# atenpas/gpd

Hardware: AMD Instinct MI355X
Metric: 15-ch grasp candidates scored/sec (imagegen+LeNet) at 1/2/4/8 MI355X (higher is better)
Workload: dtype f64 geometry / u8 images / LeNet f32-equivalent by exact operand splitting: conv1 int8 digit planes of 32-bit fixed-point weights (i32 accumulate, exact), conv2 + ip1 three bf16 pieces per operand (six exact products per term, f32 accumulate), ip2 f32

## Files before the change

gpd_amd/csrc/lenet_fast.hip:

```cpp
#include "gpd_internal.h"
#include "buffers.h"

#include <cstring>

namespace gpd {

typedef int i32x4 __attribute__((ext_vector_type(4)));
typedef float f32x4 __attribute__((ext_vector_type(4)));
typedef __bf16 bf16x8 __attribute__((ext_vector_type(8)));
typedef unsigned int u32x4 __attribute__((ext_vector_type(4)));

constexpr int F1_THREADS = 512, F1_WAVES = 8;
constexpr int F1_PITCH = 72;
constexpr int F1_ROWB = F1_PITCH * 16;
constexpr int F1_HWC = kImg * F1_ROWB;
constexpr int F1_TILES = 28 * 7;
constexpr int F1_KS = 7, F1_MT = 5;

__host__ __device__ constexpr int f1_tap(int ks, int g) {
  return ks < 5 ? ((g == 0 ? 0 : g == 1 ? 2 : g == 2 ? 1 : 3) * 5 + ks) : ks == 5 ? 20 + g : (g == 0 ? 24 : -1);
}
constexpr int F1P_KS = 5;
constexpr int F1P_ROWB = 736;
constexpr int F1P_COPY = kImg * F1P_ROWB;
constexpr int F1N_KS = 3;
constexpr int F1N_PITCH = 68;
constexpr int F1N_COPY = kImg * F1N_PITCH * 4;
__host__ __device__ constexpr int f1n_slot(int ks, int g) {
  const int sl = 4 * ks + g;
  return sl < 5 ? 2 * sl : sl < 10 ? 2 * (sl - 5) + 1 : -1;
}

__device__ inline double max_f64(double a, double b) {
  double r;
  asm("v_max_f64 %0, %1, %2" : "=v"(r) : "v"(a), "v"(b));
  return r;
}
__device__ inline double dpp_quad_max(double v) {
  int lo = __double2loint(v), hi = __double2hiint(v);
  double o = __hiloint2double(__builtin_amdgcn_mov_dpp(hi, 0xB1, 0xf, 0xf, true), __builtin_amdgcn_mov_dpp(lo, 0xB1, 0xf, 0xf, true));
  v = max_f64(v, o);
  lo = __double2loint(v);
  hi = __double2hiint(v);
  o = __hiloint2double(__builtin_amdgcn_mov_dpp(hi, 0x4E, 0xf, 0xf, true), __builtin_amdgcn_mov_dpp(lo, 0x4E, 0xf, 0xf, true));
  return max_f64(v, o);
}

template <int C, bool RELU>
__device__ __forceinline__ void conv1_i8_body(const uint8_t *__restrict__ images, const uint4 *__restrict__ atab,
                                              const double *__restrict__ corr, const int *__restrict__ shift,
                                              const float *__restrict__ bias, float *__restrict__ pool1, int n,
                                              int *__restrict__ queue) {
  constexpr int RAW = C * kPix, NV = RAW / 16;
  static_assert(RAW % 16 == 0 && C <= 16, "image bytes");
  constexpr bool NARROW = C <= 4;
  constexpr bool PACK12 = C == 12;
  constexpr int KS = NARROW ? F1N_KS : PACK12 ? F1P_KS : F1_KS;
  __shared__ __attribute__((aligned(16))) uint8_t s_hwc[NARROW ? 4 * F1N_COPY : PACK12 ? 2 * F1P_COPY : F1_HWC];
  __shared__ __attribute__((aligned(16))) uint8_t s_raw[RAW];
  __shared__ int s_nxt;
  const int tid = threadIdx.x, lane = tid & 63;
  const int wave = __builtin_amdgcn_readfirstlane(tid >> 6);
  const int j = lane & 15, q = lane >> 4;
  int img = blockIdx.x;
  if (img >= n) return;
  if (wave < F1_WAVES / 2) __builtin_amdgcn_s_setprio(2);
  i32x4 A[KS][F1_MT];
#pragma unroll
  for (int ks = 0; ks < KS; ks++)
#pragma unroll
    for (int mt = 0; mt < F1_MT; mt++) {
      const uint4 v = atab[(ks * F1_MT + mt) * 64 + lane];
      A[ks][mt] = i32x4{(int)v.x, (int)v.y, (int)v.z, (int)v.w};
    }
  {
    const uint4 *src = reinterpret_cast<const uint4 *>(images + (size_t)img * RAW);
    uint4 *dst = reinterpret_cast<uint4 *>(s_raw);
    for (int i = tid; i < NV; i += F1_THREADS) dst[i] = src[i];
  }
  __syncthreads();
  auto transpose = [&]() {
    if constexpr (NARROW) {
      for (int task = tid; task < kImg * (kImg / 4); task += F1_THREADS) {
        const int y = task / (kImg / 4), x0 = 4 * (task - y * (kImg / 4));
        uint32_t r[4];
#pragma unroll
        for (int c = 0; c < 4; c++) r[c] = c < C ? *reinterpret_cast<const uint32_t *>(s_raw + c * kPix + y * kImg + x0) : 0x80808080u;
        const uint32_t t0 = __builtin_amdgcn_perm(r[1], r[0], 0x05010400u), t1 = __builtin_amdgcn_perm(r[1], r[0], 0x07030602u);
        const uint32_t t2 = __builtin_amdgcn_perm(r[3], r[2], 0x05010400u), t3 = __builtin_amdgcn_perm(r[3], r[2], 0x07030602u);
        const uint32_t o0 = __builtin_amdgcn_perm(t2, t0, 0x05040100u) ^ 0x80808080u, o1 = __builtin_amdgcn_perm(t2, t0, 0x07060302u) ^ 0x80808080u;
        const uint32_t o2 = __builtin_amdgcn_perm(t3, t1, 0x05040100u) ^ 0x80808080u, o3 = __builtin_amdgcn_perm(t3, t1, 0x07060302u) ^ 0x80808080u;
        uint8_t *d = s_hwc + (y * F1N_PITCH + x0) * 4;
        *reinterpret_cast<uint4 *>(d) = make_uint4(o0, o1, o2, o3);
#pragma unroll
        for (int sh = 1; sh < 4; sh++) {
          uint32_t *e = reinterpret_cast<uint32_t *>(d + sh * F1N_COPY + sh * 4);
          e[0] = o0;
          e[1] = o1;
          e[2] = o2;
          e[3] = o3;
        }
      }
      return;
    }
    if constexpr (PACK12) {
      for (int task = tid; task < kImg * (kImg / 4); task += F1_THREADS) {
        const int y = task / (kImg / 4), x0 = 4 * (task - y * (kImg / 4));
        uint32_t o[4][3];
#pragma unroll
        for (int cg = 0; cg < 3; cg++) {
          uint32_t r[4];
#pragma unroll
          for (int c = 0; c < 4; c++) r[c] = *reinterpret_cast<const uint32_t *>(s_raw + (4 * cg + c) * kPix + y * kImg + x0);
          const uint32_t t0 = __builtin_amdgcn_perm(r[1], r[0], 0x05010400u), t1 = __builtin_amdgcn_perm(r[1], r[0], 0x07030602u);
          const uint32_t t2 = __builtin_amdgcn_perm(r[3], r[2], 0x05010400u), t3 = __builtin_amdgcn_perm(r[3], r[2], 0x07030602u);
          o[0][cg] = __builtin_amdgcn_perm(t2, t0, 0x05040100u) ^ 0x80808080u;
          o[1][cg] = __builtin_amdgcn_perm(t2, t0, 0x07060302u) ^ 0x80808080u;
          o[2][cg] = __builtin_amdgcn_perm(t3, t1, 0x05040100u) ^ 0x80808080u;
          o[3][cg] = __builtin_amdgcn_perm(t3, t1, 0x07060302u) ^ 0x80808080u;
        }
        uint8_t *d = s_hwc + y * F1P_ROWB + 12 * x0;
        uint4 *d4 = reinterpret_cast<uint4 *>(d);
        d4[0] = make_uint4(o[0][0], o[0][1], o[0][2], o[1][0]);
        d4[1] = make_uint4(o[1][1], o[1][2], o[2][0], o[2][1]);
        d4[2] = make_uint4(o[2][2], o[3][0], o[3][1], o[3][2]);
        uint32_t *e = reinterpret_cast<uint32_t *>(d + F1P_COPY + 4);
#pragma unroll
        for (int px = 0; px < 4; px++)
#pragma unroll
          for (int cg = 0; cg < 3; cg++) e[3 * px + cg] = o[px][cg];
      }
      return;
    }
    for (int task = tid; task < kImg * (kImg / 4); task += F1_THREADS) {
      const int y = task / (kImg / 4), x0 = 4 * (task - y * (kImg / 4));
      uint32_t r[16];
#pragma unroll
      for (int c = 0; c < 16; c++) r[c] = c < C ? *reinterpret_cast<const uint32_t *>(s_raw + c * kPix + y * kImg + x0) : 0u;
      uint32_t o[4][4];
#pragma unroll
      for (int cg = 0; cg < 4; cg++) {
        const uint32_t t0 = __builtin_amdgcn_perm(r[4 * cg + 1], r[4 * cg], 0x05010400u);
        const uint32_t t1 = __builtin_amdgcn_perm(r[4 * cg + 1], r[4 * cg], 0x07030602u);
        const uint32_t t2 = __builtin_amdgcn_perm(r[4 * cg + 3], r[4 * cg + 2], 0x05010400u);
        const uint32_t t3 = __builtin_amdgcn_perm(r[4 * cg + 3], r[4 * cg + 2], 0x07030602u);
        o[0][cg] = __builtin_amdgcn_perm(t2, t0, 0x05040100u) ^ 0x80808080u;
        o[1][cg] = __builtin_amdgcn_perm(t2, t0, 0x07060302u) ^ 0x80808080u;
        o[2][cg] = __builtin_amdgcn_perm(t3, t1, 0x05040100u) ^ 0x80808080u;
        o[3][cg] = __builtin_amdgcn_perm(t3, t1, 0x07060302u) ^ 0x80808080u;
      }
#pragma unroll
      for (int e = 0; e < 4; e++)
        *reinterpret_cast<uint4 *>(s_hwc + (y * F1_PITCH + x0 + e) * 16) = make_uint4(o[e][0], o[e][1], o[e][2], o[e][3]);
    }
  };
  transpose();
  const int m_row = (j >> 1) & 1, m_x = 2 * (j >> 2) + (j & 1);
  const int kyg = q == 0 ? 0 : q == 1 ? 2 : q == 2 ? 1 : 3;
  const int n_shift = (4 - (m_x & 3)) & 3;
  const int lane_off = NARROW   ? n_shift * F1N_COPY + (m_row * F1N_PITCH + m_x + n_shift) * 4
                       : PACK12 ? (m_x & 1) * (F1P_COPY + 4) + m_row * F1P_ROWB + 12 * m_x + 16 * q
                                : (m_row * F1_PITCH + m_x) * 16;
  int n_slot[F1N_KS];
#pragma unroll
  for (int ks = 0; ks < F1N_KS; ks++) {
    const int sl = q == 0 ? f1n_slot(ks, 0) : q == 1 ? f1n_slot(ks, 1) : q == 2 ? f1n_slot(ks, 2) : f1n_slot(ks, 3);
    n_slot[ks] = sl < 0 ? 0 : ((sl >> 1) * F1N_PITCH + 4 * (sl & 1)) * 4;
  }
  const int p = j & 3, w = j >> 2;
  const double k_corr_own = corr[4 * p + q], k_corr_4 = corr[16 + q];
  const int k_shift_own = shift[4 * p + q], k_shift_4 = shift[16 + q];
  const float k_bias_own = bias[4 * p + q], k_bias_4 = bias[16 + q];
  for (;;) {
    if (tid == 0) s_nxt = (int)gridDim.x + atomicAdd(queue, 1);
    __syncthreads();
    const int nxt = s_nxt;
    const uint4 *nsrc = reinterpret_cast<const uint4 *>(images + (size_t)(nxt < n ? nxt : img) * RAW);
    auto tile_addr = [&](int t, const uint8_t *&pa, const uint8_t *&pb, const uint8_t *&pc) {
      const int tc = t < F1_TILES ? t : F1_TILES - 1;
      const int trow = tc / 7, tcol = tc - 7 * trow;
      if constexpr (NARROW) {
        pa = pb = pc = s_hwc + ((2 * trow) * F1N_PITCH + 8 * tcol) * 4 + lane_off;
      } else if constexpr (PACK12) {
        pa = pb = pc = s_hwc + (2 * trow) * F1P_ROWB + 12 * (8 * tcol) + lane_off;
      } else {
        const uint8_t *base = s_hwc + ((2 * trow) * F1_PITCH + 8 * tcol) * 16 + lane_off;
        pa = base + kyg * F1_ROWB;
        pb = base + 4 * F1_ROWB + q * 16;
        pc = base + 4 * F1_ROWB + 4 * 16;
      }
    };
    auto frag_b = [&](int ks, const uint8_t *pa, const uint8_t *pb, const uint8_t *pc) {
      if constexpr (NARROW) return *reinterpret_cast<const i32x4 *>(pa + n_slot[ks < F1N_KS ? ks : 0]);
      else if constexpr (PACK12) {
        typedef const volatile __attribute__((address_space(3))) unsigned long long *lds_u64;
        const unsigned long long lo = *(lds_u64)(pa + ks * F1P_ROWB), hi = *(lds_u64)(pa + ks * F1P_ROWB + 8);
        return i32x4{(int)(uint32_t)lo, (int)(uint32_t)(lo >> 32), (int)(uint32_t)hi, (int)(uint32_t)(hi >> 32)};
      }
      else return *reinterpret_cast<const i32x4 *>(ks < 5 ? pa + ks * 16 : ks == 5 ? pb : pc);
    };
    i32x4 B[KS];
    {
      const uint8_t *pa, *pb, *pc;
      tile_addr(wave, pa, pb, pc);
#pragma unroll
      for (int ks = 0; ks < KS; ks++) B[ks] = frag_b(ks, pa, pb, pc);
    }
    int it = 0;
    for (int t = wave; t < F1_TILES; t += F1_WAVES, it++) {
      const int piece = it * F1_THREADS + tid;
      const bool has_piece = nxt < n && piece < NV;
      uint4 stage = make_uint4(0, 0, 0, 0);
      if (has_piece) stage = nsrc[piece];
      i32x4 acc[F1_MT];
#pragma unroll
      for (int mt = 0; mt < F1_MT; mt++) acc[mt] = i32x4{0, 0, 0, 0};
      __builtin_amdgcn_sched_barrier(0);
#pragma unroll
      for (int ks = 0; ks < KS; ks++)
#pragma unroll
        for (int mt = 0; mt < F1_MT; mt++) acc[mt] = __builtin_amdgcn_mfma_i32_16x16x64_i8(A[ks][mt], B[ks], acc[mt], 0, 0, 0);
      __builtin_amdgcn_sched_barrier(0);
      {
        const uint8_t *pa, *pb, *pc;
        tile_addr(t + F1_WAVES, pa, pb, pc);
#pragma unroll
        for (int ks = 0; ks < KS; ks++) B[ks] = frag_b(ks, pa, pb, pc);
      }
      __builtin_amdgcn_sched_barrier(0);
      double sm[F1_MT];
#pragma unroll
      for (int mt = 0; mt < F1_MT; mt++) {
        const int hi = (int)((unsigned)acc[mt][3] << 8) + acc[mt][2];
        const int lo = (int)((unsigned)acc[mt][1] << 8) + acc[mt][0];
        sm[mt] = dpp_quad_max(__builtin_fma((double)hi, 65536.0, (double)lo));
      }
      const double s_own = p == 0 ? sm[0] : p == 1 ? sm[1] : p == 2 ? sm[2] : sm[3];
      float v_own = ldexpf((float)(s_own + k_corr_own), -k_shift_own) + k_bias_own;
      float v_4 = ldexpf((float)(sm[4] + k_corr_4), -k_shift_4) + k_bias_4;
      if constexpr (RELU) {
        v_own = fmaxf(v_own, 0.f);
        v_4 = fmaxf(v_4, 0.f);
      }
      const int trow = t / 7, tcol = t - 7 * trow;
      float *dst = pool1 + ((size_t)img * 784 + trow * 28 + 4 * tcol + w) * 20;
      dst[4 * p + q] = v_own;
      if (p == 0) dst[16 + q] = v_4;
      if (has_piece) reinterpret_cast<uint4 *>(s_raw)[piece] = stage;
    }
    __syncthreads();
    if (nxt >= n) break;
    transpose();
    img = nxt;
  }
}

template <int C>
__global__ __launch_bounds__(F1_THREADS) void conv1_i8_kernel(const uint8_t *__restrict__ images,
                                                              const uint4 *__restrict__ atab, const double *__restrict__ corr,
                                                              const int *__restrict__ shift, const float *__restrict__ bias,
                                                              float *__restrict__ pool1, int n, int *__restrict__ queue) {
  conv1_i8_body<C, false>(images, atab, corr, shift, bias, pool1, n, queue);
}
template <int C>
__global__ __launch_bounds__(F1_THREADS) void conv1_i8_relu_kernel(const uint8_t *__restrict__ images,
                                                                   const uint4 *__restrict__ atab,
                                                                   const double *__restrict__ corr,
                                                                   const int *__restrict__ shift,
                                                                   const float *__restrict__ bias, float *__restrict__ pool1,
                                                                   int n, int *__restrict__ queue) {
  conv1_i8_body<C, true>(images, atab, corr, shift, bias, pool1, n, queue);
}

__device__ inline bf16x8 as_bf16x8(const uint4 &v) {
  bf16x8 r;
  __builtin_memcpy(&r, &v, 16);
  return r;
}

struct Bf3 {
  unsigned short h, m, l;
};
__host__ __device__ inline unsigned short bf16_bits(float x) {
#if defined(__HIP_DEVICE_COMPILE__)
  const __bf16 b = (__bf16)x;
  unsigned short u;
  __builtin_memcpy(&u, &b, 2);
  return u;
#else
  uint32_t u;
  memcpy(&u, &x, 4);
  if ((u & 0x7f800000u) == 0x7f800000u) return (unsigned short)((u >> 16) | ((u & 0xffffu) ? 0x40u : 0u));
  u += 0x7fffu + ((u >> 16) & 1u);
  return (unsigned short)(u >> 16);
#endif
}
__host__ __device__ inline float bf16_value(unsigned short b) {
  const uint32_t u = (uint32_t)b << 16;
  float f;
#if defined(__HIP_DEVICE_COMPILE__)
  __builtin_memcpy(&f, &u, 4);
#else
  memcpy(&f, &u, 4);
#endif
  return f;
}
__host__ __device__ inline Bf3 bf16_split3(float a) {
  Bf3 r;
  r.h = bf16_bits(a);
  const float r1 = a - bf16_value(r.h);
  r.m = bf16_bits(r1);
  const float r2 = r1 - bf16_value(r.m);
  r.l = bf16_bits(r2);
  return r;
}

constexpr int F2_THREADS = 512;
constexpr int F2_PP = 28 * 40;
constexpr int F2_RS = 3 * F2_PP;
constexpr int F2_IMG = 28 * F2_RS;
constexpr int F2_RAW = 784 * 20 * 4;
constexpr int F2_LUNITS = 24;
constexpr int F2_XLD = kLenetXld;

constexpr int F3_KSTEPS = F2_XLD / 32;
__host__ __device__ inline size_t f3_blocked(int r, int k, int pc) {
  const int rr = r & 15;
  return ((((size_t)(r >> 4) * F3_KSTEPS + (k >> 5)) * 3 + pc) << 10) + rr * 64 + ((((k >> 3) & 3) ^ ((4 - (rr >> 2)) & 3)) << 4) + (k & 7) * 2;
}

__host__ __device__ constexpr int f2_slot_tap(int e, int g) {
  return e < 25 ? (e / 5) * 5 + g : e < 30 ? g * 5 + 4 : e == 30 ? 24 : (g == 0 ? 24 : -1);
}
__host__ __device__ constexpr int f2_slot_cg(int e, int g) { return e < 25 ? e % 5 : e < 30 ? e - 25 : e == 30 ? g : 4; }

template <bool RELU>
__device__ __forceinline__ void conv2_bf16_body(const float *__restrict__ pool1, const uint4 *__restrict__ btab,
                                                const float *__restrict__ bias, unsigned short *__restrict__ xs, int n,
                                                int *__restrict__ queue) {
  __shared__ __attribute__((aligned(16))) uint8_t s_img[F2_IMG];
  __shared__ __attribute__((aligned(16))) uint8_t s_raw[F2_RAW];
  __shared__ int s_nxt;
  const int tid = threadIdx.x, lane = tid & 63;
  const int wave = __builtin_amdgcn_readfirstlane(tid >> 6);
  const int j = lane & 15, q = lane >> 4;
  const int img0 = blockIdx.x;
  if (img0 >= n) return;
  {
    const uint4 *src = reinterpret_cast<const uint4 *>(pool1 + (size_t)img0 * (784 * 20));
    uint4 *dst = reinterpret_cast<uint4 *>(s_raw);
    for (int i = tid; i < F2_RAW / 16; i += F2_THREADS) dst[i] = src[i];
  }
  __syncthreads();
  auto split = [&]() {
    for (int task = tid; task < 784 * 5; task += F2_THREADS) {
      const int px = task / 5, cg = task - 5 * px;
      const int row = px / 28, col = px - 28 * row;
      const float4 a = *reinterpret_cast<const float4 *>(s_raw + px * 80 + cg * 16);
      const Bf3 s0 = bf16_split3(a.x), s1 = bf16_split3(a.y), s2 = bf16_split3(a.z), s3 = bf16_split3(a.w);
      uint8_t *d = s_img + row * F2_RS + col * 40 + cg * 8;
      *reinterpret_cast<uint2 *>(d) = make_uint2(s0.h | ((uint32_t)s1.h << 16), s2.h | ((uint32_t)s3.h << 16));
      *reinterpret_cast<uint2 *>(d + F2_PP) = make_uint2(s0.m | ((uint32_t)s1.m << 16), s2.m | ((uint32_t)s3.m << 16));
      *reinterpret_cast<uint2 *>(d + 2 * F2_PP) = make_uint2(s0.l | ((uint32_t)s1.l << 16), s2.l | ((uint32_t)s3.l << 16));
    }
  };
  split();
  auto store_x = [&](int img, int pixel, int f, float v) {
    const Bf3 sp = bf16_split3(v);
    uint8_t *o = reinterpret_cast<uint8_t *>(xs) + f3_blocked(img, pixel * 50 + f, 0);
    *reinterpret_cast<unsigned short *>(o) = sp.h;
    *reinterpret_cast<unsigned short *>(o + 1024) = sp.m;
    *reinterpret_cast<unsigned short *>(o + 2048) = sp.l;
  };
  auto image_loop = [&](int passes, auto carries, auto &&work) {
    int img = img0;
    for (;;) {
      if (tid == 0) s_nxt = (int)gridDim.x + atomicAdd(queue, 1);
      __syncthreads();
      const int nxt = s_nxt;
      const uint4 *nsrc = reinterpret_cast<const uint4 *>(pool1 + (size_t)(nxt < n ? nxt : img) * (784 * 20));
#pragma unroll 1
      for (int tt = 0; tt < passes; tt++) {
        const int piece = tt * (7 * 64) + tid;
        const bool has_piece = decltype(carries)::value && nxt < n && piece < F2_RAW / 16;
        uint4 stage = make_uint4(0, 0, 0, 0);
        if (has_piece) stage = nsrc[piece];
        work(img, tt);
        if (has_piece) reinterpret_cast<uint4 *>(s_raw)[piece] = stage;
      }
      __syncthreads();
      if (nxt >= n) break;
      split();
      img = nxt;
    }
  };
  if (wave == 7) {
    __builtin_amdgcn_s_setprio(3);
    bf16x8 LW[3][4];
#pragma unroll
    for (int pc = 0; pc < 3; pc++)
#pragma unroll
      for (int ks = 0; ks < 4; ks++) LW[pc][ks] = as_bf16x8(btab[((3 * 3 + pc) * 16 + ks) * 64 + lane]);
    int l_lo[4], l_hi[4];
#pragma unroll
    for (int ks = 0; ks < 4; ks++) {
      const int idx = min(4 * ks + q, 14), ky = idx / 3, c8 = idx - 3 * ky;
      l_lo[ks] = ky * F2_RS + j * 40 + c8 * 16;
      l_hi[ks] = c8 == 2 ? l_lo[ks] : l_lo[ks] + 8;
    }
    const int f_own = 48 + (q & 1);
    const float k_bias = bias[f_own];
    auto unit_base = [&](int u) { return s_img + (2 * (u >> 1)) * F2_RS + (12 * (u & 1)) * 40; };
    auto lfrag = [&](const uint8_t *ubase, int step, int pc) -> bf16x8 {
      typedef const volatile __attribute__((address_space(3))) unsigned long long *lds_u64;
      const uint8_t *a = ubase + (step >> 2) * F2_RS + pc * F2_PP;
      const unsigned long long lo = *(lds_u64)(a + l_lo[step & 3]), hi = *(lds_u64)(a + l_hi[step & 3]);
      return as_bf16x8(make_uint4((uint32_t)lo, (uint32_t)(lo >> 32), (uint32_t)hi, (uint32_t)(hi >> 32)));
    };
    bf16x8 b_buf[4][3];
    auto shl = [](float v, auto n) {
      return __builtin_bit_cast(float, __builtin_amdgcn_update_dpp(0, __builtin_bit_cast(int, v), 0x100 + decltype(n)::value, 0xf, 0xf, true));
    };
    asm volatile("" ::"v"(k_bias));
    image_loop(F2_LUNITS, std::false_type(), [&](int img, int tt) {
      const uint8_t *ubase = unit_base(tt), *unext = unit_base(tt < F2_LUNITS - 1 ? tt + 1 : tt);
      if (tt == 0) {
#pragma unroll
        for (int st = 0; st < 3; st++)
#pragma unroll
          for (int pc = 0; pc < 3; pc++) b_buf[st][pc] = lfrag(ubase, st, pc);
      }
      f32x4 lacc[2][2] = {{f32x4{0.f, 0.f, 0.f, 0.f}, f32x4{0.f, 0.f, 0.f, 0.f}}, {f32x4{0.f, 0.f, 0.f, 0.f}, f32x4{0.f, 0.f, 0.f, 0.f}}};
#pragma unroll
      for (int step = 0; step < 8; step++) {
#pragma unroll
        for (int pc = 0; pc < 3; pc++) b_buf[(step + 3) & 3][pc] = step + 3 < 8 ? lfrag(ubase, step + 3, pc) : lfrag(unext, step + 3 - 8, pc);
#pragma unroll
        for (int term = 0; term < 6; term++) {
          const int pa = term == 0 ? 2 : (term == 2 || term == 3) ? 1 : 0;
          const int pw = term == 1 ? 2 : (term == 2 || term == 4) ? 1 : 0;
          lacc[step >> 2][term & 1] = __builtin_amdgcn_mfma_f32_16x16x32_bf16(LW[pw][step & 3], b_buf[step & 3][pa], lacc[step >> 2][term & 1], 0, 0, 0);
        }
      }
      float conv_row[2];
#pragma unroll
      for (int rr = 0; rr < 2; rr++) {
        const f32x4 t = lacc[rr][0] + lacc[rr][1];
        const float v = ((t[0] + shl(t[1], std::integral_constant<int, 1>())) + shl(t[2], std::integral_constant<int, 2>())) + shl(t[3], std::integral_constant<int, 3>());
        conv_row[rr] = v + __shfl(shl(t[0], std::integral_constant<int, 4>()), (lane + 32) & 63);
      }
      float pv = fmaxf(conv_row[0], conv_row[1]);
      pv = fmaxf(pv, shl(pv, std::integral_constant<int, 1>())) + k_bias;
      if constexpr (RELU) pv = fmaxf(pv, 0.f);
      if (q < 2 && (j & 1) == 0 && j < 12) store_x(img, (tt >> 1) * 12 + 6 * (tt & 1) + (j >> 1), f_own, pv);
    });
    return;
  }
  const int grp = wave < 4 ? 1 + (wave >> 1) : 0;
  const int t0 = wave == 3 ? 20 : wave < 4 ? 18 * (wave & 1) : 12 * (wave - 4), tcnt = wave == 2 ? 20 : wave == 3 ? 16 : wave < 4 ? 18 : 12;
  bf16x8 W[3][16];
#pragma unroll
  for (int pc = 0; pc < 3; pc++)
#pragma unroll
    for (int ks = 0; ks < 16; ks++) W[pc][ks] = as_bf16x8(btab[((grp * 3 + pc) * 16 + ks) * 64 + lane]);
  const int m_row = (j >> 1) & 1, m_x = 2 * (j >> 2) + (j & 1);
  const int lane_off = m_row * F2_RS + m_x * 40;
  const int off_x = lane_off + 40 * q, off_y = lane_off + q * F2_RS + 4 * 40, off_z = lane_off + 4 * F2_RS + 4 * 40 + 8 * q,
            off_w = lane_off + 4 * F2_RS + 4 * 40 + 32;
  const int f_own = 16 * grp + j;
  const float k_bias = bias[f_own];
  auto tile_base = [&](int tt) {
    const int T = t0 + tt, rp = T / 3, xt = T - 3 * rp;
    return s_img + (2 * rp) * F2_RS + (8 * xt) * 40;
  };
  auto frag = [&](const uint8_t *base, int ks, int pc) -> bf16x8 {
    uint2 v[2];
#pragma unroll
    for (int h = 0; h < 2; h++) {
      const int e = ks + 16 * h;
      const uint8_t *a = e < 25 ? base + off_x + (e / 5) * F2_RS + (e % 5) * 8
                         : e < 30 ? base + off_y + (e - 25) * 8
                         : e == 30 ? base + off_z
                                   : base + off_w;
      typedef const volatile __attribute__((address_space(3))) unsigned long long *lds_u64;
      const unsigned long long t = *(lds_u64)(a + pc * F2_PP);
      v[h] = make_uint2((uint32_t)t, (uint32_t)(t >> 32));
    }
    return as_bf16x8(make_uint4(v[0].x, v[0].y, v[1].x, v[1].y));
  };
  bf16x8 a_buf[2][3];
  image_loop(tcnt, std::true_type(), [&](int img, int tt) {
    if (tt == 0) {
#pragma unroll
      for (int pc = 0; pc < 3; pc++) a_buf[0][pc] = frag(tile_base(0), 0, pc);
    }
    const int T = t0 + tt, rp = T / 3, xt = T - 3 * rp;
    const uint8_t *base = tile_base(tt), *base_next = tile_base(tt < tcnt - 1 ? tt + 1 : tt);
    f32x4 acc[2] = {f32x4{0.f, 0.f, 0.f, 0.f}, f32x4{0.f, 0.f, 0.f, 0.f}};
#pragma unroll
    for (int ks = 0; ks < 16; ks++) {
#pragma unroll
      for (int pc = 0; pc < 3; pc++) a_buf[(ks + 1) & 1][pc] = ks + 1 < 16 ? frag(base, ks + 1, pc) : frag(base_next, 0, pc);
#pragma unroll
      for (int term = 0; term < 6; term++) {
        const int pa = term == 0 ? 2 : (term == 2 || term == 3) ? 1 : 0;
        const int pw = term == 1 ? 2 : (term == 2 || term == 4) ? 1 : 0;
        acc[term & 1] = __builtin_amdgcn_mfma_f32_16x16x32_bf16(a_buf[ks & 1][pa], W[pw][ks], acc[term & 1], 0, 0, 0);
      }
    }
    const f32x4 t = acc[0] + acc[1];
    float pv = fmaxf(fmaxf(t[0], t[1]), fmaxf(t[2], t[3])) + k_bias;
    if constexpr (RELU) pv = fmaxf(pv, 0.f);
    store_x(img, rp * 12 + 4 * xt + q, f_own, pv);
  });
}

__global__ __launch_bounds__(F2_THREADS) void conv2_bf16_kernel(const float *__restrict__ pool1,
                                                                const uint4 *__restrict__ btab, const float *__restrict__ bias,
                                                                unsigned short *__restrict__ xs, int n,
                                                                int *__restrict__ queue) {
  conv2_bf16_body<false>(pool1, btab, bias, xs, n, queue);
}
__global__ __launch_bounds__(F2_THREADS) void conv2_bf16_relu_kernel(const float *__restrict__ pool1,
                                                                     const uint4 *__restrict__ btab,
                                                                     const float *__restrict__ bias,
                                                                     unsigned short *__restrict__ xs, int n,
                                                                     int *__restrict__ queue) {
  conv2_bf16_body<true>(pool1, btab, bias, xs, n, queue);
}

constexpr int F3_THREADS = 512, F3_BN = 256, F3_BK = 32, F3_KQ = 4;
constexpr int F3_KLEN = F2_XLD / F3_KQ, F3_STEPS = F3_KLEN / F3_BK;
static_assert(F2_XLD % (F3_KQ * F3_BK) == 0 && F2_XLD >= kFc1In, "K quarters");
static_assert(F3_STEPS % 2 == 1, "the step loop below runs in pairs + one");

typedef const __attribute__((address_space(1))) void *glds_src_t;
typedef __attribute__((address_space(3))) void *glds_dst_t;

template <int NT>
__global__ __launch_bounds__(F3_THREADS) void fc1_bf16_kernel(const unsigned short *__restrict__ xs, const unsigned short *__restrict__ wt,
                                                             float *__restrict__ out_p, int n) {
  constexpr int BM = 32 * NT;
  constexpr int XB = BM * 64, WB = F3_BN * 64;
  constexpr int STAGE = 3 * (XB + WB);
  __shared__ __attribute__((aligned(16))) uint8_t smem_a[STAGE];
  __shared__ __attribute__((aligned(16))) uint8_t smem_b[STAGE];
  static_assert(2 * STAGE <= 160 * 1024, "LDS");
  const int tid = threadIdx.x;
  const int L = blockIdx.x;
  const int xcd = L & 7;
  const int ut = xcd & 1, kq = xcd >> 1;
  const int m0 = (L >> 3) * BM;
  if (m0 >= n) return;
  const int u0 = ut * F3_BN, k_base = kq * F3_KLEN;
  const int wave = __builtin_amdgcn_readfirstlane(tid >> 6), lane = tid & 63;
  const int wm = wave >> 2, wu = wave & 3;
  const int g = lane >> 4, j = lane & 15;
  constexpr int XBLK = 6 * NT, X_PW = (XBLK + 7) / 8;
  constexpr size_t ROWBLK = (size_t)F3_KSTEPS * 3 * 1024;
  const uint8_t *wsrc[2];
#pragma unroll
  for (int i = 0; i < 2; i++)
    wsrc[i] = reinterpret_cast<const uint8_t *>(wt) + (size_t)(u0 / 16 + wave + 8 * i) * ROWBLK + (size_t)(k_base / 32) * 3072 + lane * 16;
  const uint8_t *xsrc[X_PW];
  int xdst[X_PW];
#pragma unroll
  for (int i = 0; i < X_PW; i++) {
    const int e = min(wave + 8 * i, XBLK - 1), rb = e / 3, pc = e - 3 * rb;
    xsrc[i] = reinterpret_cast<const uint8_t *>(xs) + (size_t)min(m0 / 16 + rb, (n - 1) / 16) * ROWBLK + (size_t)(k_base / 32) * 3072 + pc * 1024 + lane * 16;
    xdst[i] = pc * XB + rb * 1024;
  }
  auto fetch = [&](int step, uint8_t *b) {
    const int so = step * 3072;
#pragma unroll
    for (int pc = 0; pc < 3; pc++)
#pragma unroll
      for (int i = 0; i < 2; i++)
        __builtin_amdgcn_global_load_lds((glds_src_t)(wsrc[i] + so + pc * 1024), (glds_dst_t)(b + 3 * XB + pc * WB + (wave + 8 * i) * 1024), 16, 0, 0);
#pragma unroll
    for (int i = 0; i < X_PW; i++)
      if (wave + 8 * i < XBLK) __builtin_amdgcn_global_load_lds((glds_src_t)(xsrc[i] + so), (glds_dst_t)(b + xdst[i]), 16, 0, 0);
  };
  f32x4 acc[NT][4];
#pragma unroll
  for (int t = 0; t < NT; t++)
#pragma unroll
    for (int c = 0; c < 4; c++) acc[t][c] = f32x4{0.f, 0.f, 0.f, 0.f};
  const int foff = j * 64 + ((g ^ ((4 - (j >> 2)) & 3)) << 4);
  const int xoff = (wm * 16 * NT) * 64 + foff, woff = (wu * 64) * 64 + foff;
  auto compute = [&](const uint8_t *b) {
    bf16x8 wb[3][4], xa[2][NT];
    auto ldw = [&](int pc) {
#pragma unroll
      for (int c = 0; c < 4; c++) wb[pc][c] = as_bf16x8(*reinterpret_cast<const uint4 *>(b + 3 * XB + pc * WB + woff + c * 16 * 64));
    };
    auto ldx = [&](int s, int pa) {
#pragma unroll
      for (int t = 0; t < NT; t++) xa[s][t] = as_bf16x8(*reinterpret_cast<const uint4 *>(b + pa * XB + xoff + t * 16 * 64));
    };
    auto mul = [&](int s, int pw) {
#pragma unroll
      for (int t = 0; t < NT; t++)
#pragma unroll
        for (int c = 0; c < 4; c++) acc[t][c] = __builtin_amdgcn_mfma_f32_16x16x32_bf16(xa[s][t], wb[pw][c], acc[t][c], 0, 0, 0);
    };
    ldw(0);
    ldx(0, 2);
    ldw(1);
    ldx(1, 1);
    __builtin_amdgcn_sched_barrier(0);
    mul(0, 0);
    __builtin_amdgcn_sched_barrier(0);
    ldw(2);
    ldx(0, 0);
    __builtin_amdgcn_sched_barrier(0);
    mul(1, 1);
    mul(1, 0);
    __builtin_amdgcn_sched_barrier(0);
    mul(0, 2);
    mul(0, 1);
    mul(0, 0);
  };
  fetch(0, smem_a);
  __syncthreads();
  for (int t = 0; t < F3_STEPS - 1; t += 2) {
    fetch(t + 1, smem_b);
    __builtin_amdgcn_sched_barrier(0);
    compute(smem_a);
    __syncthreads();
    fetch(t + 2, smem_a);
    __builtin_amdgcn_sched_barrier(0);
    compute(smem_b);
    __syncthreads();
  }
  compute(smem_a);
#pragma unroll
  for (int c = 0; c < 4; c++) {
    const int u = u0 + 64 * wu + 16 * c + j;
    if (u >= kFc1Out) continue;
#pragma unroll
    for (int t = 0; t < NT; t++) {
      const int m = m0 + 16 * NT * wm + 16 * t + 4 * g;
      if (m < n) *reinterpret_cast<f32x4 *>(out_p + fc1p_index(m, kq, u)) = acc[t][c];
    }
  }
}

void lenet_fast_free(LeNetFast &f) {
  device_release(f.c1a, f.c1corr, f.c1shift, f.c2b, f.f1wt);
  f = LeNetFast();
}

void lenet_fast_conv1_tables(int channels, const float *w, std::vector<uint8_t> &atab, std::vector<double> &corr, std::vector<int> &shift) {
  const int K = channels * 25;
  std::vector<long long> W((size_t)20 * K);
  corr.assign(20, 0.0);
  shift.assign(20, 0);
  for (int f = 0; f < 20; f++) {
    float mx = 0.f;
    for (int k = 0; k < K; k++) mx = std::fmax(mx, std::fabs(w[(size_t)f * K + k]));
    int s = 0;
    if (mx > 0.f) {
      int e;
      (void)std::frexp(mx, &e);
      s = 30 - e;
    }
    shift[f] = s;
    long long sum = 0;
    for (int k = 0; k < K; k++) {
      const long long v = std::llrint(std::ldexp((double)w[(size_t)f * K + k], s));
      W[(size_t)f * K + k] = v;
      sum += v;
    }
    corr[f] = 128.0 * (double)sum;
  }
  atab.assign((size_t)F1_KS * F1_MT * 64 * 16, 0);
  auto digit_of = [](long long v, int digit) {
    int d = 0;
    for (int q = 0; q <= digit; q++) {
      d = (int)(((v + 128) & 255) - 128);
      v = (v - d) >> 8;
    }
    return d;
  };
  const bool narrow = channels <= 4;
  const bool pack12 = channels == 12;
  for (int ks = 0; ks < (narrow ? F1N_KS : pack12 ? F1P_KS : F1_KS); ks++)
    for (int mt = 0; mt < F1_MT; mt++)
      for (int lane = 0; lane < 64; lane++) {
        const int i = lane & 15, g = lane >> 4;
        const int f = 4 * mt + (i >> 2), digit = i & 3;
        uint8_t *row = &atab[((size_t)(ks * F1_MT + mt) * 64 + lane) * 16];
        if (narrow) {
          const int sl = f1n_slot(ks, g);
          if (sl < 0) continue;
          const int ky = sl >> 1, half = sl & 1;
          for (int px = 0; px < 4; px++) {
            const int kx = 4 * half + px;
            if (kx > 4) continue;
            for (int c = 0; c < channels; c++) row[4 * px + c] = (uint8_t)(int8_t)digit_of(W[(size_t)f * K + c * 25 + ky * 5 + kx], digit);
          }
          continue;
        }
        if (pack12) {
          for (int b = 0; b < 16; b++) {
            const int kb = 16 * g + b;
            if (kb >= 60) continue;
            row[b] = (uint8_t)(int8_t)digit_of(W[(size_t)f * K + (kb % 12) * 25 + ks * 5 + kb / 12], digit);
          }
          continue;
        }
        const int tap = f1_tap(ks, g);
        if (tap < 0) continue;
        for (int c = 0; c < channels; c++) row[c] = (uint8_t)(int8_t)digit_of(W[(size_t)f * K + c * 25 + tap], digit);
      }
}

void lenet_fast_conv2_tables(const float *w, std::vector<unsigned short> &btab) {
  btab.assign((size_t)4 * 3 * 16 * 64 * 8, 0);
  auto put = [&](int slot, int ks, int lane, int e, float v) {
    const Bf3 sp = bf16_split3(v);
    const unsigned short pcs[3] = {sp.h, sp.m, sp.l};
    for (int pc = 0; pc < 3; pc++) btab[((((size_t)slot * 3 + pc) * 16 + ks) * 64 + lane) * 8 + e] = pcs[pc];
  };
  for (int slot = 0; slot < 3; slot++)
    for (int ks = 0; ks < 16; ks++)
      for (int lane = 0; lane < 64; lane++) {
        const int f = 16 * slot + (lane & 15), g = lane >> 4;
        for (int h = 0; h < 2; h++) {
          const int e = ks + 16 * h, tap = f2_slot_tap(e, g), cg = f2_slot_cg(e, g);
          if (tap < 0) continue;
          for (int c = 0; c < 4; c++) put(slot, ks, lane, 4 * h + c, w[(size_t)f * 500 + (4 * cg + c) * 25 + tap]);
        }
      }
  for (int ks = 0; ks < 4; ks++)
    for (int lane = 0; lane < 64; lane++) {
      const int row = lane & 15, chunk = 4 * ks + (lane >> 4);
      if ((row > 8 && row != 12) || chunk > 14) continue;
      const int f = row < 8 ? 48 + (row >> 2) : 48 + ((row - 8) >> 2), kx = row < 8 ? (row & 3) : 4;
      const int ky = chunk / 3, c0 = 8 * (chunk % 3);
      for (int e = 0; e < 8 && c0 + e < 20; e++) put(3, ks, lane, e, w[(size_t)f * 500 + (c0 + e) * 25 + ky * 5 + kx]);
    }
}

void lenet_fast_ip1_tables(const float *w, std::vector<unsigned short> &wt) {
  wt.assign((size_t)3 * 512 * F2_XLD, 0);
  uint8_t *base = reinterpret_cast<uint8_t *>(wt.data());
  for (int k = 0; k < kFc1In; k++)
    for (int u = 0; u < kFc1Out; u++) {
      const Bf3 sp = bf16_split3(w[(size_t)k * kFc1Out + u]);
      const unsigned short pcs[3] = {sp.h, sp.m, sp.l};
      for (int pc = 0; pc < 3; pc++) memcpy(base + f3_blocked(u, k, pc), &pcs[pc], 2);
    }
}

void lenet_fast_unblock_x(const unsigned short *blocked, int n, unsigned short *planes) {
  const uint8_t *base = reinterpret_cast<const uint8_t *>(blocked);
  for (int pc = 0; pc < 3; pc++)
    for (int m = 0; m < n; m++)
      for (int k = 0; k < kFc1In; k++) memcpy(planes + ((size_t)pc * n + m) * kFc1In + k, base + f3_blocked(m, k, pc), 2);
}

}

extern "C" int gpd_hip_lenet_fast_tables(int channels, const float *c1w, const float *c2w, uint8_t *atab, double *corr, int *shift,
                                         unsigned short *btab) {
  if (!c1w || !c2w || !atab || !corr || !shift || !btab || channels < 1 || channels > 16) return GPD_ERR_INVALID;
  std::vector<uint8_t> a;
  std::vector<double> c;
  std::vector<int> sh;
  std::vector<unsigned short> b;
  gpd::lenet_fast_conv1_tables(channels, c1w, a, c, sh);
  gpd::lenet_fast_conv2_tables(c2w, b);
  memcpy(atab, a.data(), a.size());
  memcpy(corr, c.data(), c.size() * sizeof(double));
  memcpy(shift, sh.data(), sh.size() * sizeof(int));
  memcpy(btab, b.data(), b.size() * sizeof(unsigned short));
  return GPD_OK;
}

namespace gpd {

hipError_t lenet_fast_prepare(LeNetFast &f, int channels, const float *c1w, const float *c2w, const float *f1w) {
  lenet_fast_free(f);
  std::vector<uint8_t> atab;
  std::vector<double> corr;
  std::vector<int> shift;
  std::vector<unsigned short> btab, wt;
  lenet_fast_conv1_tables(channels, c1w, atab, corr, shift);
  lenet_fast_conv2_tables(c2w, btab);
  lenet_fast_ip1_tables(f1w, wt);
  hipError_t e;
  auto up = [&](auto *&dst, const void *src, size_t bytes) -> hipError_t {
    if ((e = device_alloc(dst, (bytes + sizeof(*dst) - 1) / sizeof(*dst))) != hipSuccess) return e;
    return hipMemcpy(dst, src, bytes, hipMemcpyHostToDevice);
  };
  if ((e = up(f.c1a, atab.data(), atab.size())) != hipSuccess) return e;
  if ((e = up(f.c1corr, corr.data(), corr.size() * sizeof(double))) != hipSuccess) return e;
  if ((e = up(f.c1shift, shift.data(), shift.size() * sizeof(int))) != hipSuccess) return e;
  if ((e = up(f.c2b, btab.data(), btab.size() * sizeof(unsigned short))) != hipSuccess) return e;
  if ((e = up(f.f1wt, wt.data(), wt.size() * sizeof(unsigned short))) != hipSuccess) return e;
  return hipSuccess;
}

template <int NT>
static void fc1f_launch(const LeNetWeights &w, LeNetScratch &s, int n, hipStream_t stream) {
  const int m_tiles = (n + 32 * NT - 1) / (32 * NT);
  fc1_bf16_kernel<NT><<<m_tiles * 8, F3_THREADS, 0, stream>>>(s.xs, w.fast.f1wt, s.fc1p, n);
}
static int fc1f_pick_nt(int n) {
  for (int r = 1;; r++) {
    const int nt = (n + 32 * r * 32 - 1) / (32 * r * 32);
    if (nt <= 5) return nt < 1 ? 1 : nt;
  }
}

hipError_t lenet_forward_fast(const LeNetWeights &w, LeNetScratch &s, const uint8_t *img, int m, float *d_scores, hipStream_t stream,
                              hipEvent_t *kernel_events, int *queue) {
  const int num_cus = s.num_cus;
  const int grid = m < num_cus ? m : num_cus;
#define F1_LAUNCH(KERNEL, CH) KERNEL<CH><<<grid, F1_THREADS, 0, stream>>>(img, w.fast.c1a, w.fast.c1corr, w.fast.c1shift, w.c1b, s.pool1, m, queue)
  if (w.conv_relu) {
    switch (w.channels) {
      case 15: F1_LAUNCH(conv1_i8_relu_kernel, 15); break;
      case 12: F1_LAUNCH(conv1_i8_relu_kernel, 12); break;
      case 3: F1_LAUNCH(conv1_i8_relu_kernel, 3); break;
      case 1: F1_LAUNCH(conv1_i8_relu_kernel, 1); break;
      default: return hipErrorInvalidValue;
    }
  } else {
    switch (w.channels) {
      case 15: F1_LAUNCH(conv1_i8_kernel, 15); break;
      case 12: F1_LAUNCH(conv1_i8_kernel, 12); break;
      case 3: F1_LAUNCH(conv1_i8_kernel, 3); break;
      case 1: F1_LAUNCH(conv1_i8_kernel, 1); break;
      default: return hipErrorInvalidValue;
    }
  }
#undef F1_LAUNCH
  if (kernel_events) (void)hipEventRecord(kernel_events[0], stream);
  if (w.conv_relu)
    conv2_bf16_relu_kernel<<<grid, F2_THREADS, 0, stream>>>(s.pool1, w.fast.c2b, w.c2b, s.xs, m, queue + 1);
  else
    conv2_bf16_kernel<<<grid, F2_THREADS, 0, stream>>>(s.pool1, w.fast.c2b, w.c2b, s.xs, m, queue + 1);
  if (kernel_events) (void)hipEventRecord(kernel_events[1], stream);
  switch (fc1f_pick_nt(m)) {
    case 1: fc1f_launch<1>(w, s, m, stream); break;
    case 2: fc1f_launch<2>(w, s, m, stream); break;
    case 3: fc1f_launch<3>(w, s, m, stream); break;
    case 4: fc1f_launch<4>(w, s, m, stream); break;
    default: fc1f_launch<5>(w, s, m, stream); break;
  }
  if (kernel_events) (void)hipEventRecord(kernel_events[2], stream);
  return hipGetLastError();
}

}
```

Before: 2.270 million.

## Fold conv1 correction into MFMA accumulators and trim epilogue and split overheads

The conv1 correction constant is now preloaded into the int32 MFMA accumulators instead of being added in f64 afterwards. The quad max reduction drops from f64 DPP moves to f32 v_max_f32_dpp via inline asm, and pool1 stores use a scalar base plus a fixed per-lane offset. Conv2 splits two bf16 values at once with a packed vector conversion and handles two tasks per loop iteration, and the xs store address is built from a scalar per-image base. A host-side check rejects weights whose folded correction could overflow the int32 accumulators, and self-checks confirm the new address helpers match the original layout. In exchange, the max is now taken in f32 before the shift, which relies on exact rounding, and inline asm adds fragility.

New measurement: 2.312 million, median of 6. 1.8% higher.

```diff
diff --git a/gpd_amd/csrc/lenet_fast.hip b/gpd_amd/csrc/lenet_fast.hip
--- a/gpd_amd/csrc/lenet_fast.hip
+++ b/gpd_amd/csrc/lenet_fast.hip
@@ -31,19 +31,12 @@
   return sl < 5 ? 2 * sl : sl < 10 ? 2 * (sl - 5) + 1 : -1;
 }
 
-__device__ inline double max_f64(double a, double b) {
-  double r;
-  asm("v_max_f64 %0, %1, %2" : "=v"(r) : "v"(a), "v"(b));
-  return r;
-}
-__device__ inline double dpp_quad_max(double v) {
-  int lo = __double2loint(v), hi = __double2hiint(v);
-  double o = __hiloint2double(__builtin_amdgcn_mov_dpp(hi, 0xB1, 0xf, 0xf, true), __builtin_amdgcn_mov_dpp(lo, 0xB1, 0xf, 0xf, true));
-  v = max_f64(v, o);
-  lo = __double2loint(v);
-  hi = __double2hiint(v);
-  o = __hiloint2double(__builtin_amdgcn_mov_dpp(hi, 0x4E, 0xf, 0xf, true), __builtin_amdgcn_mov_dpp(lo, 0x4E, 0xf, 0xf, true));
-  return max_f64(v, o);
+__device__ __forceinline__ void dpp_quad_max5(float (&f)[5]) {
+#define GPD_QMAX(n, perm) "v_max_f32_dpp %" #n ", %" #n ", %" #n " quad_perm:" perm " row_mask:0xf bank_mask:0xf\n\t"
+  asm("s_nop 1\n\t" GPD_QMAX(0, "[1,0,3,2]") GPD_QMAX(1, "[1,0,3,2]") GPD_QMAX(2, "[1,0,3,2]") GPD_QMAX(3, "[1,0,3,2]") GPD_QMAX(4, "[1,0,3,2]")
+          GPD_QMAX(0, "[2,3,0,1]") GPD_QMAX(1, "[2,3,0,1]") GPD_QMAX(2, "[2,3,0,1]") GPD_QMAX(3, "[2,3,0,1]") GPD_QMAX(4, "[2,3,0,1]")
+      : "+v"(f[0]), "+v"(f[1]), "+v"(f[2]), "+v"(f[3]), "+v"(f[4]));
+#undef GPD_QMAX
 }
 
 template <int C, bool RELU>
@@ -168,14 +161,22 @@
     n_slot[ks] = sl < 0 ? 0 : ((sl >> 1) * F1N_PITCH + 4 * (sl & 1)) * 4;
   }
   const int p = j & 3, w = j >> 2;
-  const double k_corr_own = corr[4 * p + q], k_corr_4 = corr[16 + q];
+  i32x4 k_start[F1_MT];
+#pragma unroll
+  for (int mt = 0; mt < F1_MT; mt++) {
+    const long long c = (long long)corr[4 * mt + q];
+    const int c0 = (int)(((c + (1 << 23)) & 0xffffff) - (1 << 23));
+    k_start[mt] = i32x4{c0, 0, 0, (int)((c - c0) >> 24)};
+  }
+  const uint32_t k_voff = ((w * 20 + 4 * p + q) * 4);
   const int k_shift_own = shift[4 * p + q], k_shift_4 = shift[16 + q];
   const float k_bias_own = bias[4 * p + q], k_bias_4 = bias[16 + q];
   for (;;) {
     if (tid == 0) s_nxt = (int)gridDim.x + atomicAdd(queue, 1);
     __syncthreads();
-    const int nxt = s_nxt;
+    const int nxt = __builtin_amdgcn_readfirstlane(s_nxt);
     const uint4 *nsrc = reinterpret_cast<const uint4 *>(images + (size_t)(nxt < n ? nxt : img) * RAW);
+    const uint64_t pool_img = (uint64_t)__builtin_amdgcn_readfirstlane(img) * (784 * 20 * 4);
     auto tile_addr = [&](int t, const uint8_t *&pa, const uint8_t *&pb, const uint8_t *&pc) {
       const int tc = t < F1_TILES ? t : F1_TILES - 1;
       const int trow = tc / 7, tcol = tc - 7 * trow;
@@ -214,7 +215,7 @@
       if (has_piece) stage = nsrc[piece];
       i32x4 acc[F1_MT];
 #pragma unroll
-      for (int mt = 0; mt < F1_MT; mt++) acc[mt] = i32x4{0, 0, 0, 0};
+      for (int mt = 0; mt < F1_MT; mt++) acc[mt] = k_start[mt];
       __builtin_amdgcn_sched_barrier(0);
 #pragma unroll
       for (int ks = 0; ks < KS; ks++)
@@ -228,24 +229,27 @@
         for (int ks = 0; ks < KS; ks++) B[ks] = frag_b(ks, pa, pb, pc);
       }
       __builtin_amdgcn_sched_barrier(0);
-      double sm[F1_MT];
+      float sm[F1_MT];
 #pragma unroll
       for (int mt = 0; mt < F1_MT; mt++) {
         const int hi = (int)((unsigned)acc[mt][3] << 8) + acc[mt][2];
         const int lo = (int)((unsigned)acc[mt][1] << 8) + acc[mt][0];
-        sm[mt] = dpp_quad_max(__builtin_fma((double)hi, 65536.0, (double)lo));
-      }
-      const double s_own = p == 0 ? sm[0] : p == 1 ? sm[1] : p == 2 ? sm[2] : sm[3];
-      float v_own = ldexpf((float)(s_own + k_corr_own), -k_shift_own) + k_bias_own;
-      float v_4 = ldexpf((float)(sm[4] + k_corr_4), -k_shift_4) + k_bias_4;
+        sm[mt] = (float)__builtin_fma((double)hi, 65536.0, (double)lo);
+      }
+      dpp_quad_max5(sm);
+      const float s_own = p == 0 ? sm[0] : p == 1 ? sm[1] : p == 2 ? sm[2] : sm[3];
+      float v_own = ldexpf(s_own, -k_shift_own) + k_bias_own;
+      float v_4 = ldexpf(sm[4], -k_shift_4) + k_bias_4;
       if constexpr (RELU) {
         v_own = fmaxf(v_own, 0.f);
         v_4 = fmaxf(v_4, 0.f);
       }
       const int trow = t / 7, tcol = t - 7 * trow;
-      float *dst = pool1 + ((size_t)img * 784 + trow * 28 + 4 * tcol + w) * 20;
-      dst[4 * p + q] = v_own;
-      if (p == 0) dst[16 + q] = v_4;
+      uint8_t *const dst = reinterpret_cast<uint8_t *>(pool1) + (pool_img + (trow * 28 + 4 * tcol) * 80);
+      uint32_t voff = k_voff;
+      asm("" : "+v"(voff));
+      *reinterpret_cast<float *>(dst + voff) = v_own;
+      if (p == 0) asm volatile("global_store_dword %0, %1, %2 offset:64" ::"v"(voff), "v"(v_4), "s"(dst) : "memory");
       if (has_piece) reinterpret_cast<uint4 *>(s_raw)[piece] = stage;
     }
     __syncthreads();
@@ -315,6 +319,24 @@
   return r;
 }
 
+__host__ __device__ inline uint32_t bf16_pair_bits(float x0, float x1) {
+#if defined(__HIP_DEVICE_COMPILE__)
+  typedef float f32x2 __attribute__((ext_vector_type(2)));
+  typedef __bf16 bf16x2 __attribute__((ext_vector_type(2)));
+  return __builtin_bit_cast(uint32_t, __builtin_convertvector(f32x2{x0, x1}, bf16x2));
+#else
+  return bf16_bits(x0) | ((uint32_t)bf16_bits(x1) << 16);
+#endif
+}
+__host__ __device__ inline void bf16_split3_pair(float a0, float a1, uint32_t &h, uint32_t &m, uint32_t &l) {
+  h = bf16_pair_bits(a0, a1);
+  float r0 = a0 - bf16_value((unsigned short)h), r1 = a1 - bf16_value((unsigned short)(h >> 16));
+  m = bf16_pair_bits(r0, r1);
+  r0 -= bf16_value((unsigned short)m);
+  r1 -= bf16_value((unsigned short)(m >> 16));
+  l = bf16_pair_bits(r0, r1);
+}
+
 constexpr int F2_THREADS = 512;
 constexpr int F2_PP = 28 * 40;
 constexpr int F2_RS = 3 * F2_PP;
@@ -328,6 +350,10 @@
   const int rr = r & 15;
   return ((((size_t)(r >> 4) * F3_KSTEPS + (k >> 5)) * 3 + pc) << 10) + rr * 64 + ((((k >> 3) & 3) ^ ((4 - (rr >> 2)) & 3)) << 4) + (k & 7) * 2;
 }
+
+constexpr size_t F3_ROWBLK = (size_t)F3_KSTEPS * 3 << 10;
+__host__ __device__ inline size_t f3_row_base(int r) { return (size_t)(r >> 4) * F3_ROWBLK + (r & 15) * 64; }
+__host__ __device__ inline uint32_t f3_elem(int k, int sw) { return (uint32_t)(k >> 5) * 3072u + ((((k >> 3) & 3) ^ sw) << 4) + (k & 7) * 2; }
 
 __host__ __device__ constexpr int f2_slot_tap(int e, int g) {
   return e < 25 ? (e / 5) * 5 + g : e < 30 ? g * 5 + 4 : e == 30 ? 24 : (g == 0 ? 24 : -1);
@@ -353,21 +379,30 @@
   }
   __syncthreads();
   auto split = [&]() {
-    for (int task = tid; task < 784 * 5; task += F2_THREADS) {
+    auto put = [&](int task, const float4 &a) {
       const int px = task / 5, cg = task - 5 * px;
       const int row = px / 28, col = px - 28 * row;
-      const float4 a = *reinterpret_cast<const float4 *>(s_raw + px * 80 + cg * 16);
-      const Bf3 s0 = bf16_split3(a.x), s1 = bf16_split3(a.y), s2 = bf16_split3(a.z), s3 = bf16_split3(a.w);
+      uint32_t h0, m0, l0, h1, m1, l1;
+      bf16_split3_pair(a.x, a.y, h0, m0, l0);
+      bf16_split3_pair(a.z, a.w, h1, m1, l1);
       uint8_t *d = s_img + row * F2_RS + col * 40 + cg * 8;
-      *reinterpret_cast<uint2 *>(d) = make_uint2(s0.h | ((uint32_t)s1.h << 16), s2.h | ((uint32_t)s3.h << 16));
-      *reinterpret_cast<uint2 *>(d + F2_PP) = make_uint2(s0.m | ((uint32_t)s1.m << 16), s2.m | ((uint32_t)s3.m << 16));
-      *reinterpret_cast<uint2 *>(d + 2 * F2_PP) = make_uint2(s0.l | ((uint32_t)s1.l << 16), s2.l | ((uint32_t)s3.l << 16));
+      *reinterpret_cast<uint2 *>(d) = make_uint2(h0, h1);
+      *reinterpret_cast<uint2 *>(d + F2_PP) = make_uint2(m0, m1);
+      *reinterpret_cast<uint2 *>(d + 2 * F2_PP) = make_uint2(l0, l1);
+    };
+    for (int task = tid; task < 784 * 5; task += 2 * F2_THREADS) {
+      const int task1 = task + F2_THREADS < 784 * 5 ? task + F2_THREADS : task;
+      const float4 a0 = *reinterpret_cast<const float4 *>(s_raw + task * 16);
+      const float4 a1 = *reinterpret_cast<const float4 *>(s_raw + task1 * 16);
+      put(task, a0);
+      put(task1, a1);
     }
   };
   split();
   auto store_x = [&](int img, int pixel, int f, float v) {
     const Bf3 sp = bf16_split3(v);
-    uint8_t *o = reinterpret_cast<uint8_t *>(xs) + f3_blocked(img, pixel * 50 + f, 0);
+    const int simg = __builtin_amdgcn_readfirstlane(img);
+    uint8_t *o = reinterpret_cast<uint8_t *>(xs) + f3_row_base(simg) + f3_elem(pixel * 50 + f, (4 - ((simg & 15) >> 2)) & 3);
     *reinterpret_cast<unsigned short *>(o) = sp.h;
     *reinterpret_cast<unsigned short *>(o + 1024) = sp.m;
     *reinterpret_cast<unsigned short *>(o + 2048) = sp.l;
@@ -377,7 +412,7 @@
     for (;;) {
       if (tid == 0) s_nxt = (int)gridDim.x + atomicAdd(queue, 1);
       __syncthreads();
-      const int nxt = s_nxt;
+      const int nxt = __builtin_amdgcn_readfirstlane(s_nxt);
       const uint4 *nsrc = reinterpret_cast<const uint4 *>(pool1 + (size_t)(nxt < n ? nxt : img) * (784 * 20));
 #pragma unroll 1
       for (int tt = 0; tt < passes; tt++) {
@@ -651,7 +686,7 @@
   f = LeNetFast();
 }
 
-void lenet_fast_conv1_tables(int channels, const float *w, std::vector<uint8_t> &atab, std::vector<double> &corr, std::vector<int> &shift) {
+bool lenet_fast_conv1_tables(int channels, const float *w, std::vector<uint8_t> &atab, std::vector<double> &corr, std::vector<int> &shift) {
   const int K = channels * 25;
   std::vector<long long> W((size_t)20 * K);
   corr.assign(20, 0.0);
@@ -683,6 +718,19 @@
     }
     return d;
   };
+  bool in_bounds = true;
+  for (int f = 0; f < 20; f++) {
+    long long mag[4] = {0, 0, 0, 0};
+    for (int k = 0; k < K; k++)
+      for (int d = 0; d < 4; d++) mag[d] += std::llabs((long long)digit_of(W[(size_t)f * K + k], d));
+    if (!(std::fabs(corr[f]) < 9007199254740992.0)) {
+      in_bounds = false;
+      continue;
+    }
+    const long long c = (long long)corr[f], c0 = ((c + (1 << 23)) & 0xffffff) - (1 << 23), c3 = (c - c0) >> 24;
+    const long long hi = (128 * mag[3] + std::llabs(c3)) * 256 + 128 * mag[2], lo = 128 * mag[1] * 256 + 128 * mag[0] + std::llabs(c0);
+    if (hi >= (1ll << 31) || lo >= (1ll << 31)) in_bounds = false;
+  }
   const bool narrow = channels <= 4;
   const bool pack12 = channels == 12;
   for (int ks = 0; ks < (narrow ? F1N_KS : pack12 ? F1P_KS : F1_KS); ks++)
@@ -714,6 +762,7 @@
         if (tap < 0) continue;
         for (int c = 0; c < channels; c++) row[c] = (uint8_t)(int8_t)digit_of(W[(size_t)f * K + c * 25 + tap], digit);
       }
+  return in_bounds;
 }
 
 void lenet_fast_conv2_tables(const float *w, std::vector<unsigned short> &btab) {
@@ -770,13 +819,13 @@
   std::vector<double> c;
   std::vector<int> sh;
   std::vector<unsigned short> b;
-  gpd::lenet_fast_conv1_tables(channels, c1w, a, c, sh);
+  const bool in_bounds = gpd::lenet_fast_conv1_tables(channels, c1w, a, c, sh);
   gpd::lenet_fast_conv2_tables(c2w, b);
   memcpy(atab, a.data(), a.size());
   memcpy(corr, c.data(), c.size() * sizeof(double));
   memcpy(shift, sh.data(), sh.size() * sizeof(int));
   memcpy(btab, b.data(), b.size() * sizeof(unsigned short));
-  return GPD_OK;
+  return in_bounds ? GPD_OK : GPD_ERR_INVALID;
 }
 
 namespace gpd {
@@ -787,9 +836,14 @@
   std::vector<double> corr;
   std::vector<int> shift;
   std::vector<unsigned short> btab, wt;
-  lenet_fast_conv1_tables(channels, c1w, atab, corr, shift);
+  if (!lenet_fast_conv1_tables(channels, c1w, atab, corr, shift)) return hipErrorInvalidValue;
   lenet_fast_conv2_tables(c2w, btab);
   lenet_fast_ip1_tables(f1w, wt);
+  for (int r = 0; r < 16; r++)
+    for (int k = 0; k < F2_XLD; k++)
+      for (int pc = 0; pc < 3; pc++)
+        if (f3_row_base(r) + f3_elem(k, (4 - (r >> 2)) & 3) + ((size_t)pc << 10) != f3_blocked(r, k, pc)) return hipErrorAssert;
+  if (f3_row_base(70000 + 5) + f3_elem(7199, (4 - (5 >> 2)) & 3) != f3_blocked(70000 + 5, 7199, 0)) return hipErrorAssert;
   hipError_t e;
   auto up = [&](auto *&dst, const void *src, size_t bytes) -> hipError_t {
     if ((e = device_alloc(dst, (bytes + sizeof(*dst) - 1) / sizeof(*dst))) != hipSuccess) return e;
```
